# vtuber-plan/vcvits

Measured on AMD Instinct MI355X. Metric: training utterances/sec (gen+disc step) at base.json segment_size, higher is better.
Workload: dtype f32; 1 GPU; configs/base.json widths, HiFi-GAN generator + MPD(8 periods+S) + MSD + STFT/mel-L1, G step + D step + AdamW (learning rate 0: weights held at their seeded initial values); per_gpu_batch=16, global_batch=16, segment_size=16384, parallelism=dp1, process_group_ranks=1, graph_recording_steps_before_warmup=3

## Files before the change

include/vcvits_hip.h:

```cpp
#ifndef VCVITS_HIP_H
#define VCVITS_HIP_H

#include <stdint.h>

#ifdef __cplusplus
extern "C" {
#endif

#define VCV_OK 0
#define VCV_EINVAL (-1)
#define VCV_EHIP (-2)
#define VCV_ELDS (-3)

#define VCV_ACT_NONE 0
#define VCV_ACT_LEAKY 1
#define VCV_ACT_RELU 2
#define VCV_ACT_TANH 3
#define VCV_ACT_LOGCLAMP 4

#define VCV_TF_NONE 0
#define VCV_TF_LEAKY 1
#define VCV_TF_DLEAKY 2
#define VCV_TF_DRELU 3
#define VCV_TF_DTANH 4
// ... 71 lines not shown

typedef struct VcvWgradArgs {
  const float* a;
  const float* b;
  const float* aaux;
  const float* baux;
  float* dw;
  int32_t B, G, Cg, Mg;
  int32_t Ta, Tb, P;
  int32_t K;
  int32_t s, dj, off;
  int32_t a_tf, b_tf;
  int32_t transpose_out;
  float alpha, slope;
  float* dbias;
  float* slab;
  int64_t slab_floats;
  int32_t split_terms;
} VcvWgradArgs;

int vcv_conv_wgrad(const VcvWgradArgs* args, void* stream);
int vcv_conv_wgrad_takes_dma(const VcvWgradArgs* args);
int vcv_conv_wgrad_split_terms(const VcvWgradArgs* args);

int64_t vcv_wgrad_bf16_scratch(const VcvWgradArgs* args);
int vcv_wgrad_bf16(const VcvWgradArgs* args, float* scratch, int64_t scratch_floats, void* stream);
int64_t vcv_wgrad_x3_scratch(const VcvWgradArgs* args);
int vcv_wgrad_x3(const VcvWgradArgs* args, float* scratch, int64_t scratch_floats, void* stream);
int vcv_wgrad_bf16_set_force(int cand, int z);

int vcv_conv_m1_fwd(const float* x, const float* w, const float* bias, float* y, int B, int C, int Tin,
                    int Tout, int P, int K, int stride, int dil, int pad, int in_leaky, int out_act,
                    float slope, void* stream);
int vcv_conv_c1_fwd(const float* x, const float* w, const float* bias, float* y, int B, int M, int Tin, int Tout,
                    int P, int K, int stride, int dil, int pad, int out_act, float slope, void* stream);
int vcv_conv_c1_fwd_masked(const float* x, const float* w, const float* bias, float* y, const float* oaux, int B, int M,
                           int Tin, int Tout, int P, int K, int stride, int dil, int pad, int out_act, float slope,
                           void* stream);
int vcv_conv_c1_fwd_flip(const float* x, const float* w, const float* bias, float* y, const float* oaux, int B, int M, int Tin,
                         int Tout, int P, int K, int stride, int dil, int pad, int out_act, float slope, int flip_taps,
                         void* stream);
int vcv_conv_c1_dgrad(const float* dy, const float* w, float* dx, int B, int M, int Tin, int Tout, int P, int K,
                      int stride, int dil, int pad, void* stream);
int vcv_linear_t1_fwd(const float* x, const float* w, const float* bias, float* y, int B, int C, int M, void* stream);
int vcv_linear_t1_dgrad(const float* dy, const float* w, float* dx, int B, int C, int M, void* stream);
int vcv_linear_t1_wgrad(const float* dy, const float* x, float* dw, int B, int C, int M, void* stream);
// ... 235 lines not shown
```

vcvits_amd/_lib.py:

```python
import ctypes
import os

import torch

_HERE = os.path.dirname(os.path.abspath(__file__))
from . import tuning

LIB_PATH = tuning.text("VCVITS_HIP_LIB", "", "path of another build of libvcvits_hip.so (A/B builds)") or \
    os.path.join(_HERE, "csrc", "libvcvits_hip.so")

VCV_OK = 0
ACT_NONE, ACT_LEAKY, ACT_RELU, ACT_TANH, ACT_LOGCLAMP = 0, 1, 2, 3, 4
TF_NONE, TF_LEAKY, TF_DLEAKY, TF_DRELU, TF_DTANH, TF_DLOGCLAMP = 0, 1, 2, 3, 4, 5

_f32p = ctypes.c_void_p
_i32 = ctypes.c_int32


class VcvConvArgs(ctypes.Structure):
    _fields_ = [
        ("x", _f32p), ("w", _f32p), ("bias", _f32p), ("res", _f32p), ("mask", _f32p),
        ("xaux", _f32p), ("oaux", _f32p), ("y", _f32p),
        ("B", _i32), ("G", _i32), ("Cg", _i32), ("Mg", _i32),
        ("Tin", _i32), ("Tout", _i32), ("P", _i32),
# ... 40 lines not shown


def lib():
    global _lib
    if _lib is None:
        if not os.path.exists(LIB_PATH):
            raise RuntimeError(
                "libvcvits_hip.so not found at %s -- run `python -m vcvits_amd.build_ext` "
                "(there is no CPU fallback for the vcvits hot path)" % LIB_PATH)
        L = ctypes.CDLL(LIB_PATH)
        L.vcv_version.restype = ctypes.c_char_p
        for name in EXPORTS:
            fn = getattr(L, name)
            if name != "vcv_version":
                fn.restype = (ctypes.c_int64 if name in ("vcv_conv_dma_workspace", "vcv_wgrad_bf16_scratch", "vcv_wgrad_x3_scratch", "vcv_layernorm_c_bwd_scratch", "vcv_resblock_pair_supported",
                                                                "vcv_rel_attn_stream_bwd_workspace")
                              else ctypes.c_void_p if name == "vcv_get_seed_offset_ptr" else ctypes.c_int)
                fn.argtypes = _ARGTYPES[name]
        _lib = L
    return _lib


EXPORTS = [
    "vcv_version", "vcv_conv_gemm", "vcv_conv_wgrad", "vcv_conv_wgrad_takes_dma", "vcv_conv_wgrad_split_terms", "vcv_bias_grad",
    "vcv_weight_norm_fwd", "vcv_weight_norm_bwd", "vcv_spectral_norm_fwd", "vcv_spectral_norm_bwd", "vcv_avg3", "vcv_scale", "vcv_mask_mul",
    "vcv_reflect_pad_fwd", "vcv_reflect_pad_bwd", "vcv_avgpool4_fwd", "vcv_avgpool4_bwd",
    "vcv_loss_sum", "vcv_loss_grad", "vcv_adamw", "vcv_stft_mag_fwd", "vcv_stft_mag_bwd",
    "vcv_wn_gate_fwd", "vcv_wn_gate_bwd", "vcv_row_sum", "vcv_wn_res_skip_fwd", "vcv_wn_res_skip_bwd",
    "vcv_split_sample_fwd", "vcv_split_sample_bwd", "vcv_coupling", "vcv_layernorm_c_fwd",
    "vcv_layernorm_c_bwd", "vcv_rel_softmax_fwd", "vcv_rel_value_fwd", "vcv_rel_softmax_bwd",
    "vcv_kl_fwd", "vcv_kl_bwd", "vcv_nearest_fwd", "vcv_nearest_bwd", "vcv_nearest_raw_fwd", "vcv_nearest_raw_bwd", "vcv_slice_fwd", "vcv_slice_bwd",
    "vcv_dropout", "vcv_prof_begin", "vcv_prof_end", "vcv_prof_dump", "vcv_conv_m1_fwd", "vcv_conv_c1_fwd", "vcv_conv_c1_fwd_masked", "vcv_conv_c1_fwd_flip", "vcv_conv_c1_dgrad", "vcv_linear_t1_fwd", "vcv_linear_t1_dgrad", "vcv_linear_t1_wgrad", "vcv_thin_wgrad", "vcv_weight_flip_transpose",
    "vcv_act_grad", "vcv_act_grad_add", "vcv_weight_norm_many_fwd", "vcv_weight_norm_many_bwd", "vcv_loss_many_sum", "vcv_loss_many_grad", "vcv_conv_dma_workspace", "vcv_conv_dma", "vcv_conv_dma_plan", "vcv_conv_dma_run", "vcv_stft_complex_fwd", "vcv_istft", "vcv_grouped41_fwd", "vcv_grouped41_fwd_bf16", "vcv_grouped41_dgrad", "vcv_grouped41_dgrad_bf16", "vcv_grouped41_wgrad", "vcv_grouped41_wgrad_bf16",
    "vcv_prior_sample", "vcv_prof_bytes", "vcv_conv_bf16_plan", "vcv_conv_bf16_run", "vcv_wgrad_bf16_scratch", "vcv_wgrad_bf16", "vcv_act_grad_bias", "vcv_conv_pk_plan", "vcv_conv_pk_run",
    "vcv_conv_x3_plan", "vcv_conv_x3_run", "vcv_conv_x3_set_terms", "vcv_conv_x3_get_terms", "vcv_conv_x3_set_all", "vcv_wgrad_x3_scratch", "vcv_wgrad_x3", "vcv_rel_attn_supported", "vcv_rel_attn_fwd", "vcv_rel_attn_bwd", "vcv_rel_attn_bwd2", "vcv_set_deterministic", "vcv_get_deterministic", "vcv_prof_roof", "vcv_prof_pause", "vcv_conv_x3_pack_job", "vcv_conv_pk_pack_job", "vcv_conv_bf16_pack_job", "vcv_pack_many", "vcv_upload_table",
    "vcv_conv_bf16io_plan", "vcv_conv_bf16io_run", "vcv_cast_f32_x16", "vcv_cast_x16_f32", "vcv_conv_m1_x16_fwd",
    "vcv_prof_active", "vcv_set_seed_offset_ptr", "vcv_get_seed_offset_ptr", "vcv_pack_many_prepared", "vcv_adamw_dev", "vcv_set_words", "vcv_tuning_set", "vcv_tuning_get", "vcv_embedding_t_fwd", "vcv_embedding_t_fwd_checked", "vcv_embedding_t_bwd", "vcv_conv_x3_set_variant", "vcv_conv_plan_describe", "vcv_wgrad_bf16_set_force", "vcv_layernorm_c_bwd_scratch", "vcv_layernorm_c_bwd_ws", "vcv_resblock_pair_supported", "vcv_resblock_pair_pack", "vcv_resblock_pair_x16",
    "vcv_pyin_yin", "vcv_pyin_obs", "vcv_pyin_viterbi",
    "vcv_resample_table", "vcv_resample_apply", "vcv_phase_vocoder", "vcv_istft_ordered",
    "vcv_hubert_bias_gelu", "vcv_hubert_groupnorm_gelu", "vcv_hubert_layernorm_c_gelu", "vcv_hubert_attn_supported", "vcv_hubert_attn_fwd",
    "vcv_hubert_groupnorm_gelu_len", "vcv_hubert_mask_frames", "vcv_hubert_attn_fwd_len",
    "vcv_rel_attn_stream_supported", "vcv_rel_attn_stream_fwd",
    "vcv_rel_attn_stream_train_fwd", "vcv_rel_attn_stream_bwd_workspace", "vcv_rel_attn_stream_bwd",
    "vcv_rel_attn_stream_fwd_bf16", "vcv_hubert_attn_fwd_bf16", "vcv_hubert_attn_fwd_len_bf16",
]


_P, _I, _L, _F, _D = ctypes.c_void_p, ctypes.c_int, ctypes.c_int64, ctypes.c_float, ctypes.c_double
_ARGTYPES = {
    "vcv_conv_gemm": [ctypes.POINTER(VcvConvArgs), _P],
    "vcv_conv_wgrad": [ctypes.POINTER(VcvWgradArgs), _P],
    "vcv_conv_wgrad_takes_dma": [ctypes.POINTER(VcvWgradArgs)],
    "vcv_conv_wgrad_split_terms": [ctypes.POINTER(VcvWgradArgs)],
    "vcv_bias_grad": [_P, _P, _P, _I, _I, _I, _I, _F, _I, _P],
    "vcv_weight_norm_fwd": [_P, _P, _P, _P, _I, _I, _P],
    "vcv_weight_norm_bwd": [_P, _P, _P, _P, _P, _P, _I, _I, _P],
    "vcv_spectral_norm_fwd": [_P, _P, _P, _P, _P, _P, _I, _I, _I, _F, _P],
    "vcv_spectral_norm_bwd": [_P, _P, _P, _P, _P, _P, _P, _I, _I, _P],
    "vcv_avg3": [_P, _P, _P, _P, _L, _P],
    "vcv_scale": [_P, _P, _F, _L, _P],
    "vcv_mask_mul": [_P, _P, _P, _I, _I, _I, _P],
    "vcv_reflect_pad_fwd": [_P, _P, _I, _I, _I, _P],
    "vcv_reflect_pad_bwd": [_P, _P, _I, _I, _I, _P],
    "vcv_avgpool4_fwd": [_P, _P, _I, _I, _P],
    "vcv_avgpool4_bwd": [_P, _P, _I, _I, _P],
    "vcv_loss_sum": [_P, _P, _F, _I, _F, _P, _L, _P],
    "vcv_loss_grad": [_P, _P, _F, _I, _F, _P, _P, _I, _L, _P],
    "vcv_adamw": [_P, _P, _P, _P, _L, _F, _F, _F, _F, _F, _I, _P],
    "vcv_stft_mag_fwd": [_P, _P, _P, _P, _I, _I, _I, _I, _I, _I, _F, _P],
    "vcv_stft_mag_bwd": [_P, _P, _P, _P, _P, _I, _I, _I, _I, _I, _I, _F, _P],
    "vcv_wn_gate_fwd": [_P, _P, _I, _I, _P, _I, _I, _I, _P],
    "vcv_wn_gate_bwd": [_P, _P, _I, _I, _P, _P, _I, _I, _I, _P],
    "vcv_row_sum": [_P, _P, _I, _I, _I, _I, _I, _P],
    "vcv_wn_res_skip_fwd": [_P, _P, _P, _P, _P, _P, _I, _I, _I, _I, _P],
    "vcv_wn_res_skip_bwd": [_P, _P, _P, _P, _P, _I, _I, _I, _P],
    "vcv_split_sample_fwd": [_P, _P, _P, _P, _P, _P, _I, _I, _I, _P],
# ... 250 lines not shown
```

vcvits_amd/csrc/tuning.h:

```cpp
#pragma once

struct VcvTuning {
  int xcd_remap = 1;
  int pk_ws = 1;
  int pk_ws_bf16 = 0;
  int pk_x4 = 1;
  int pk_vec = 1;
  int x3_variant = -1;
  int x3_v6 = 1;
  int x3_js2 = 1;
  int x3_merge_phases = 1;
  int x3_old_ks = 0;
  int x3_all = 0;
  int x3_terms = 6;
  int wgrad_dma = 1;
  int wgrad_tile = -1;
  int wgrad_verbose = 0;
  int wgrad_dma_split = 1;
  int wgrad_bf16_ws = 1;
  int wgrad_finish_vec = 1;
  int bias_rows = 1;
  int c1_chunk = 0;
  int m1_lds = 1;
  int c1_wgrad_pairs = 1;
  int thin_wgrad_wgs = 2048;
  int act_grad_vec = 1;
  int ln_regs = 1;
  int stft_wave = 1;
  int attn_rows = 1;
  int zero_memset = 0;
  int pack_tile = 1;
  int pack_tile_bf16 = 1;
  int pair_dbg = 0;
  int pair_grid = 0;
  int pair_stream = 1;
  int deterministic = 0;
};

VcvTuning& vcv_tuning();
extern "C" int vcv_tuning_set(const char* key, int value);
extern "C" int vcv_tuning_get(const char* key, int* value);
// ... 1 lines not shown
```

vcvits_amd/csrc/version.hip:

```cpp
#include "common.h"
#include <cstring>
extern "C" const char* vcv_version(void) {
  return "vcvits_hip gfx950 fp32-mfma(32x32x2) conv family; built " __DATE__ " " __TIME__;
}

extern "C" int vcv_set_deterministic(int on) {
  vcv_tuning().deterministic = on ? 1 : 0;
  return VCV_OK;
}
extern "C" int vcv_get_deterministic(void) { return vcv_tuning().deterministic; }

namespace {
struct TuningKey { const char* name; int VcvTuning::*field; };
#define TK(f) {#f, &VcvTuning::f}
const TuningKey kTuningKeys[] = {
    TK(xcd_remap), TK(pk_ws), TK(pk_ws_bf16), TK(pk_x4), TK(pk_vec), TK(x3_variant), TK(x3_v6), TK(x3_js2), TK(x3_merge_phases), TK(x3_old_ks), TK(x3_all),
    TK(x3_terms), TK(wgrad_dma), TK(wgrad_tile), TK(wgrad_verbose), TK(wgrad_dma_split), TK(wgrad_bf16_ws), TK(wgrad_finish_vec), TK(bias_rows),
    TK(c1_chunk), TK(m1_lds), TK(c1_wgrad_pairs), TK(thin_wgrad_wgs), TK(act_grad_vec), TK(ln_regs), TK(stft_wave), TK(attn_rows),
    TK(zero_memset), TK(pack_tile), TK(pack_tile_bf16), TK(pair_dbg), TK(pair_grid), TK(pair_stream), TK(deterministic)};
#undef TK
int VcvTuning::*find_key(const char* key, size_t len) {
  for (const TuningKey& k : kTuningKeys)
    if (strlen(k.name) == len && strncmp(k.name, key, len) == 0) return k.field;
  return nullptr;
}
VcvTuning make_tuning() {
  VcvTuning t;
  const char* det = getenv("VCVITS_DETERMINISTIC");
  if (det && det[0] == '1') t.deterministic = 1;
  const char* e = getenv("VCVITS_TUNING");
  while (e && *e) {
    const char* end = strchr(e, ',');
    const size_t n = end ? (size_t)(end - e) : strlen(e);
    const char* eq = (const char*)memchr(e, '=', n);
    if (eq) {
      int VcvTuning::*f = find_key(e, (size_t)(eq - e));
      if (f) t.*f = atoi(eq + 1);
      else fprintf(stderr, "vcvits_hip: VCVITS_TUNING: unknown key '%.*s'\n", (int)(eq - e), e);
    } else if (n) {
      fprintf(stderr, "vcvits_hip: VCVITS_TUNING: '%.*s' is not key=value\n", (int)n, e);
// ... 31 lines not shown
```

vcvits_amd/csrc/wgrad_dma.hip:

```cpp
#include "common.h"
#include "prof.h"
#include "split_terms.h"
#include <cstring>
#include <unordered_map>

namespace {

constexpr int BU = 64, AP = BU + 4, MAXX = 12, TABN = BU + 32;

struct WgGeom {
  int NCH, CP, emin, G4, nmt, nnt, Z, nchunk_u, buf_floats, a_floats, tab_floats;
  float invG4, invP;
};

template <int OFF>
__device__ __forceinline__ f32x4 lds_rd128(unsigned addr) {
  f32x4 v;
  asm volatile("ds_read_b128 %0, %1 offset:%2" : "=v"(v) : "v"(addr), "n"(OFF) : "memory");
  return v;
}
__device__ __forceinline__ float lds_rd32(unsigned addr) {
  float v;
  asm volatile("ds_read_b32 %0, %1" : "=v"(v) : "v"(addr) : "memory");
  return v;
}
__device__ __forceinline__ void lds_wait() { asm volatile("s_waitcnt lgkmcnt(0)" ::: "memory"); }
__device__ __forceinline__ void pin(f32x4& f) { asm volatile("" : "+v"(f)); }
__device__ __forceinline__ void pin(float& f) { asm volatile("" : "+v"(f)); }
__device__ __forceinline__ void pin(bf16x8& f) { asm volatile("" : "+v"(f)); }
template <typename T, int N>
__device__ __forceinline__ void pin(T (&f)[N]) {
#pragma unroll
  for (int i = 0; i < N; ++i) pin(f[i]);
}
__device__ __forceinline__ void divmod(int n, int d, float inv, int& q, int& r) {
  q = (int)((float)n * inv);
  r = n - q * d;
  if (r < 0) r += d, --q;
  if (r >= d) r -= d, ++q;
}
__device__ __forceinline__ f32x4 ld128(__amdgpu_buffer_rsrc_t r, unsigned voff) {
  return __builtin_bit_cast(f32x4, __builtin_amdgcn_raw_buffer_load_b128(r, voff, 0, 0));
}

__device__ __forceinline__ void split_frag(const float (&f)[8], bf16x8 (&t)[3]) {
#pragma unroll
  for (int e = 0; e < 8; ++e) {
    __bf16 t0, t1, t2;
    split3(f[e], t0, t1, t2);
    t[0][e] = t0, t[1][e] = t1, t[2][e] = t2;
  }
}

template <int TM, int TN, int WM, int WN, bool LA, bool LB, bool BIAS, bool STR, int ST>
__global__ void __launch_bounds__(64 * (WM * WN + (WM * WN >= 8 ? 4 : 2)))
wgrad_dma_kernel(const VcvWgradArgs p, const WgGeom tg) {
  constexpr int BM = 32 * TM * WM, BN = 32 * TN * WN, NW = WM * WN, NP = NW >= 8 ? 4 : 2;
  constexpr int MAXA = BM / (4 * NP);
  extern __shared__ float smem[];
  const int tid = threadIdx.x, lane = tid & 63;
  const int wave = __builtin_amdgcn_readfirstlane(tid >> 6);
  const int l31 = lane & 31, h = lane >> 5;

  const int nt = blockIdx.x, mt = blockIdx.y, z = blockIdx.z;
  const int K = p.K, Cg = p.Cg, Mg = p.Mg, P = p.P;
  const int N = Cg * K;
  const int n0 = nt * BN, m0 = mt * BM;
  const int cfirst = n0 / K;
  const int CP = tg.CP, NCH = tg.NCH;
  const unsigned lds0 = (unsigned)(size_t)(__attribute__((address_space(3))) float*)smem;
  const int U = p.Ta * P, TbP = p.Tb * P;
  const int total = p.B * tg.nchunk_u;
  if (z >= total) return;
  auto xspan0 = [&](int uc0) __attribute__((always_inline)) {
    return STR ? ((uc0 / P) * p.s + tg.emin) * P : uc0 + tg.emin * P;
  };

  if (wave >= NW) {
    const int pw = wave - NW;
    __builtin_amdgcn_s_setprio(3);
    f32x4 ra[MAXA], rx[MAXX];
    const int ngx = NCH * tg.G4;
    int xld[MAXX], xi4[MAXX];
    unsigned xst[MAXX];
#pragma unroll
    for (int t = 0; t < MAXX; ++t) {
      const int idx = (t * NP + pw) * 64 + lane;
      int cl, i4;
      divmod(idx, tg.G4, tg.invG4, cl, i4);
      xi4[t] = 4 * i4;
      xld[t] = idx < ngx ? cl * TbP + 4 * i4 : 0x20000000;
      xst[t] = (unsigned)(idx < ngx ? tg.a_floats + cl * CP + 4 * i4 : tg.a_floats + tg.tab_floats + NCH * CP) * 4u;
    }
    if (STR && pw == 1 && lane < TABN - BU) {
      asm volatile("ds_write_b32 %0, %1" ::"v"(lds0 + (unsigned)(tg.a_floats + NCH * CP + BU + lane) * 4u), "v"(0) : "memory");
      asm volatile("ds_write_b32 %0, %1" ::"v"(lds0 + (unsigned)(tg.buf_floats + tg.a_floats + NCH * CP + BU + lane) * 4u), "v"(0)
                   : "memory");
    }
    auto store = [&](int ch, int buf) __attribute__((always_inline)) {
      const int b = ch / tg.nchunk_u;
      const int uc0 = (ch - b * tg.nchunk_u) * BU;
      const unsigned base = lds0 + (unsigned)(buf * tg.buf_floats) * 4u;
      const bool tail = uc0 + BU > U;
#pragma unroll
      for (int t = 0; t < MAXA; ++t) {
        const int row = (t * NP + pw) * 4 + (lane >> 4), c4 = lane & 15;
        f32x4 v = ra[t];
        if (tail) {
          const int nv = U - uc0 - 4 * c4;
#pragma unroll
          for (int e = 0; e < 4; ++e) v[e] = e < nv ? v[e] : 0.f;
        }
        asm volatile("ds_write_b128 %0, %1" ::"v"(base + (unsigned)(row * AP + 4 * c4) * 4u), "v"(v) : "memory");
      }
      const int f0 = xspan0(uc0), f0a = f0 & ~3;
      if (STR && pw == 0) {
        int q, pc;
        divmod(uc0 + lane, P, tg.invP, q, pc);
        const int off = ((q - uc0 / P) * p.s * P + pc + (f0 - f0a)) * 4;
        asm volatile("ds_write_b32 %0, %1" ::"v"(base + (unsigned)(tg.a_floats + NCH * CP + lane) * 4u), "v"(uc0 + lane < U ? off : 0)
                     : "memory");
      }
      const bool edge = f0a < 0 || f0a + 4 * tg.G4 > TbP;
#pragma unroll
      for (int t = 0; t < MAXX; ++t) {
        if ((t * NP + pw) * 64 < ngx) {
          f32x4 v = rx[t];
          if (edge) {
            const int f = f0a + xi4[t];
#pragma unroll
            for (int e = 0; e < 4; ++e) v[e] = (unsigned)(f + e) < (unsigned)TbP ? v[e] : 0.f;
          }
          asm volatile("ds_write_b128 %0, %1" ::"v"(base + xst[t]), "v"(v) : "memory");
        }
      }
    };
// ... 11 lines not shown
      __amdgpu_buffer_rsrc_t rX = __builtin_amdgcn_make_buffer_rsrc((void*)(p.b + ((size_t)b * Cg + cfirst) * (size_t)TbP), 0,
                                                                    (int)((size_t)(Cg - cfirst) * TbP * 4), 0x00020000);
#pragma unroll
      for (int t = 0; t < MAXX; ++t)
        if ((t * NP + pw) * 64 < ngx) {
          unsigned voff = (unsigned)(xld[t] + f0a) * 4u;
          asm volatile("" : "+v"(voff));
          rx[t] = ld128(rX, voff);
        }
    };
    load(z);
    store(z, 0);
    if (z + tg.Z < total) load(z + tg.Z);
    int bufi = 0;
    for (int ch = z; ch < total; ch += tg.Z) {
      lds_wait();
      __syncthreads();
      if (ch + tg.Z < total) {
        store(ch + tg.Z, bufi ^ 1);
        if (ch + 2 * tg.Z < total) load(ch + 2 * tg.Z);
      }
      bufi ^= 1;
    }
    return;
  }

  const int wm = wave / WN, wn = wave % WN;
  unsigned aofs[TM], nofs[TN];
#pragma unroll
  for (int tm = 0; tm < TM; ++tm) aofs[tm] = (unsigned)(((wm * TM + tm) * 32 + l31) * AP + 4 * h) * 4u;
#pragma unroll
  for (int tn = 0; tn < TN; ++tn) {
    int n = n0 + (wn * TN + tn) * 32 + l31;
    if (n > N - 1) n = N - 1;
    const int c = n / K, kw = n - c * K;
    const int e = kw * p.dj + p.off - tg.emin;
    nofs[tn] = (unsigned)(tg.a_floats + (c - cfirst) * CP + e * P + (STR ? 0 : ((tg.emin * P) & 3) + 4 * h)) * 4u;
  }
  const unsigned tabofs = (unsigned)(tg.a_floats + NCH * CP + 4 * h) * 4u;

  f32x16 acc[TM][TN];
#pragma unroll
  for (int tm = 0; tm < TM; ++tm)
#pragma unroll
    for (int tn = 0; tn < TN; ++tn)
#pragma unroll
      for (int e = 0; e < 16; ++e) acc[tm][tn][e] = 0.f;
  const bool do_bias = BIAS && nt == 0 && wn == 0;
  float bsum[TM];
#pragma unroll
  for (int tm = 0; tm < TM; ++tm) bsum[tm] = 0.f;

  int bufi = 0;
  for (int ch = z; ch < total; ch += tg.Z) {
    __syncthreads();
    const unsigned base = lds0 + (unsigned)(bufi * tg.buf_floats) * 4u;
    const int uc0 = (ch % tg.nchunk_u) * BU;
    const int rem = U - uc0;
    const int npair = rem >= BU ? BU / 16 : (rem + 15) >> 4;
    unsigned aad[TM], bad[TN], tad = base + tabofs;
#pragma unroll
    for (int tm = 0; tm < TM; ++tm) aad[tm] = base + aofs[tm];
#pragma unroll
    for (int tn = 0; tn < TN; ++tn) bad[tn] = base + nofs[tn];


    if constexpr (ST == 6) {
      f32x4 a0[TM], a1[TM], b0[TN], b1[TN], t0, t1;
      float b0s[TN][4], b1s[TN][4];
      auto rd_group = [&]() __attribute__((always_inline)) {
        if (STR) t0 = lds_rd128<0>(tad), t1 = lds_rd128<32>(tad);
#pragma unroll
        for (int tm = 0; tm < TM; ++tm) a0[tm] = lds_rd128<0>(aad[tm]), a1[tm] = lds_rd128<32>(aad[tm]);
        if (STR) {
          asm volatile("s_waitcnt lgkmcnt(%0)" ::"n"(2 * TM) : "memory");
          pin(t0), pin(t1);
        }
#pragma unroll
        for (int tn = 0; tn < TN; ++tn) {
          if (!STR) {
            b0[tn] = lds_rd128<0>(bad[tn]), b1[tn] = lds_rd128<32>(bad[tn]);
          } else {
#pragma unroll
            for (int e = 0; e < 4; ++e) b0s[tn][e] = lds_rd32(bad[tn] + __float_as_uint(t0[e]));
#pragma unroll
            for (int e = 0; e < 4; ++e) b1s[tn][e] = lds_rd32(bad[tn] + __float_as_uint(t1[e]));
          }
        }
      };
      auto settle = [&]() __attribute__((always_inline)) {
        lds_wait();
        pin(a0), pin(a1);
        if (STR) {
#pragma unroll
          for (int tn = 0; tn < TN; ++tn)
#pragma unroll
            for (int e = 0; e < 4; ++e) pin(b0s[tn][e]), pin(b1s[tn][e]);
        } else {
          pin(b0), pin(b1);
        }
      };
      rd_group();
      settle();
      for (int pr = 0; pr < npair; ++pr) {
        bf16x8 ap[TM][3], bp[TN][3];
#pragma unroll
        for (int tm = 0; tm < TM; ++tm) {
          float f[8];
#pragma unroll
          for (int e = 0; e < 4; ++e) f[e] = a0[tm][e], f[4 + e] = a1[tm][e];
          if (LA) {
#pragma unroll
            for (int e = 0; e < 8; ++e) f[e] = fmaxf(f[e], f[e] * p.slope);
          }
          if (BIAS && do_bias) bsum[tm] += ((f[0] + f[1]) + (f[2] + f[3])) + ((f[4] + f[5]) + (f[6] + f[7]));
          split_frag(f, ap[tm]);
        }
#pragma unroll
        for (int tn = 0; tn < TN; ++tn) {
          float f[8];
#pragma unroll
          for (int e = 0; e < 4; ++e) f[e] = STR ? b0s[tn][e] : b0[tn][e], f[4 + e] = STR ? b1s[tn][e] : b1[tn][e];
          if (LB) {
#pragma unroll
            for (int e = 0; e < 8; ++e) f[e] = fmaxf(f[e], f[e] * p.slope);
          }
          split_frag(f, bp[tn]);
        }
#pragma unroll
        for (int pl = 0; pl < 3; ++pl) {
#pragma unroll
          for (int tm = 0; tm < TM; ++tm) pin(ap[tm][pl]);
#pragma unroll
          for (int tn = 0; tn < TN; ++tn) pin(bp[tn][pl]);
        }
#pragma unroll
        for (int tm = 0; tm < TM; ++tm) aad[tm] += 64;
        if (!STR) {
#pragma unroll
          for (int tn = 0; tn < TN; ++tn) bad[tn] += 64;
        }
        tad += 64;
        if (pr + 1 < npair) rd_group();
        mma_product<6>(acc, ap, bp);
        settle();
      }
      bufi ^= 1;
      continue;
    }
    f32x4 a0[TM], a1[TM], b0[TN], b1[TN], t0, t1;
    float b0s[TN][4], b1s[TN][4];
#define WG_LOAD(A, Bf, T, OFF)                                                                  \
  {                                                                                             \
    _Pragma("unroll") for (int tm = 0; tm < TM; ++tm) A[tm] = lds_rd128<OFF>(aad[tm]);          \
    if (!STR) {                                                                                 \
      _Pragma("unroll") for (int tn = 0; tn < TN; ++tn) Bf[tn] = lds_rd128<OFF>(bad[tn]);       \
    } else {                                                                                    \
      _Pragma("unroll") for (int tn = 0; tn < TN; ++tn) _Pragma("unroll") for (int e = 0; e < 4; ++e)  \
          Bf##s[tn][e] = lds_rd32(bad[tn] + __float_as_uint(T[e]));                             \
    }                                                                                           \
// ... 77 lines not shown
        else unsafeAtomicAdd(p.dw + (size_t)ml * N + n, p.alpha * acc[tm][tn][e]);
      }
    }
  }
}

__global__ void __launch_bounds__(256) wgrad_slab_finish_kernel(const float* __restrict__ slab, float* __restrict__ dw,
                                                                size_t n, int Z, float alpha) {
  const size_t i = (size_t)blockIdx.x * 256 + threadIdx.x;
  if (i >= n) return;
  float s = slab[i];
  for (int z = 1; z < Z; ++z) s += slab[(size_t)z * n + i];
  dw[i] += alpha * s;
}

template <int TM, int TN, int WM, int WN, bool STR, int ST>
void (*pick_kernel_st(const VcvWgradArgs& a))(const VcvWgradArgs, const WgGeom) {
  const bool la = a.a_tf == VCV_TF_LEAKY, lb = a.b_tf == VCV_TF_LEAKY;
  return la ? (lb ? wgrad_dma_kernel<TM, TN, WM, WN, true, true, false, STR, ST> : wgrad_dma_kernel<TM, TN, WM, WN, true, false, false, STR, ST>)
            : (a.dbias ? (lb ? wgrad_dma_kernel<TM, TN, WM, WN, false, true, true, STR, ST> : wgrad_dma_kernel<TM, TN, WM, WN, false, false, true, STR, ST>)
                       : (lb ? wgrad_dma_kernel<TM, TN, WM, WN, false, true, false, STR, ST> : wgrad_dma_kernel<TM, TN, WM, WN, false, false, false, STR, ST>));
}
template <int TM, int TN, int WM, int WN, bool STR>
void (*pick_kernel(const VcvWgradArgs& a, bool split))(const VcvWgradArgs, const WgGeom) {
  return split ? pick_kernel_st<TM, TN, WM, WN, STR, 6>(a) : pick_kernel_st<TM, TN, WM, WN, STR, 0>(a);
}

constexpr double SPLIT_SHAPE[7] = {1.0, 0.83, 0.65, 0.73, 0.67, 0.57, 0.57};
constexpr double SPLIT_BASE = 0.85;

bool wanted_split(const VcvWgradArgs& a) { return (long long)a.B * a.Ta * a.P >= 1024; }

bool takes_split(const VcvWgradArgs& a) {
  const VcvTuning& t = vcv_tuning();
  return a.split_terms == 6 && t.wgrad_dma_split != 0 && t.x3_terms == 6 && (t.x3_all != 0 || wanted_split(a));
}

struct WgPlan {
  WgGeom g;
  size_t lds;
  double cost;
};

template <int TM, int TN, int WM, int WN, bool STR>
WgPlan plan(const VcvWgradArgs& a, bool split) {
  constexpr int BM = 32 * TM * WM, BN = 32 * TN * WN, NP = WM * WN >= 8 ? 4 : 2, NT = 64 * (WM * WN + NP);
  WgPlan pl;
  pl.cost = -1.0;
  WgGeom& g = pl.g;
  const int N = a.Cg * a.K;
  g.nnt = vcv_cdiv(N, BN);
  g.nmt = vcv_cdiv(a.Mg, BM);
  g.NCH = (BN - 1) / a.K + 2;
  if (g.NCH > a.Cg + 1) g.NCH = a.Cg + 1;
  const int jspan = (a.K - 1) * a.dj;
  g.emin = a.off + (jspan < 0 ? jspan : 0);
  const int emax = jspan < 0 ? -jspan : jspan;
  const int nq = STR ? (a.P - 1 + BU - 1) / a.P + 1 : 0;
  const int span = STR ? ((nq - 1) * a.s + emax + 1) * a.P : BU + emax * a.P;
  g.G4 = (span + 3 + 3) / 4;
  g.invG4 = 1.0f / (float)g.G4, g.invP = 1.0f / (float)a.P;
  if ((long long)g.NCH * g.G4 > (long long)MAXX * NP * 64) return pl;
  g.a_floats = BM * AP;
  g.tab_floats = TABN;
  int want = (a.K * (emax / (a.K > 1 ? a.K - 1 : 1)) * a.P + 3) / 4 * 4 % 64;
  if (want < 8) want = 8;
  g.CP = 4 * g.G4;
  while (g.CP % 64 != want % 64) g.CP += 4;
  if (g.CP - 4 * g.G4 > 32) g.CP = 4 * g.G4 + 4;
  for (int attempt = 0; attempt < 2; ++attempt) {
    g.buf_floats = g.a_floats + g.NCH * g.CP + g.tab_floats + 16;
    pl.lds = 2ull * g.buf_floats * 4;
    if (pl.lds <= VCV_LDS_LIMIT) break;
    g.CP = 4 * g.G4 + ((4 * g.G4) % 32 == 0 ? 4 : 0);
  }
  if (pl.lds > VCV_LDS_LIMIT) return pl;
  const long long U = (long long)a.Ta * a.P;
  g.nchunk_u = (int)((U + BU - 1) / BU);
  const long long total = (long long)a.B * g.nchunk_u;
  void (*kern)(const VcvWgradArgs, const WgGeom) = pick_kernel<TM, TN, WM, WN, STR>(a, split);
  static int occ_cache[2][2][2][2] = {};
  int& oc = occ_cache[split][a.a_tf == VCV_TF_LEAKY][a.b_tf == VCV_TF_LEAKY][a.dbias != nullptr];
  if (oc == 0) {
    (void)hipFuncSetAttribute((const void*)kern, hipFuncAttributeMaxDynamicSharedMemorySize, VCV_LDS_LIMIT);
    int nb = 0;
    if (hipOccupancyMaxActiveBlocksPerMultiprocessor(&nb, (const void*)kern, NT, 0) != hipSuccess || nb < 1) nb = 1;
    oc = nb;
  }
  long long occ = (long long)(VCV_LDS_LIMIT / pl.lds);
  if (occ > oc) occ = oc;
  if (occ < 1) occ = 1;
  const double shape = BM == 128 ? (BN == 256 ? 1.0 : BN == 128 ? 0.93 : 0.77)
                     : BM == 64  ? (BN == 256 ? 0.905 : BN == 128 ? 0.76 : 0.58)
                                 : 0.62;
  const double shape6 = BM == 128 ? (BN == 256 ? SPLIT_SHAPE[0] : BN == 128 ? SPLIT_SHAPE[1] : SPLIT_SHAPE[2])
                      : BM == 64  ? (BN == 256 ? SPLIT_SHAPE[3] : BN == 128 ? SPLIT_SHAPE[4] : SPLIT_SHAPE[5])
                                  : SPLIT_SHAPE[6];
  const double rate = (split ? SPLIT_BASE * shape6 : 0.70 * shape) * (STR ? 0.93 : 1.0) * 157.3e12 / 256.0;
  const double t_stage = 2.0 * BM * BN * BU / rate * 1e6, t_fix = 4.0;
  const long long tiles = (long long)g.nnt * g.nmt;
  const long long slots = 256 * occ;
  const size_t nw = (size_t)a.Mg * N;
  const long long zcap = a.slab ? (long long)(a.slab_floats / (int64_t)nw) : 1024;
  if (a.slab && zcap < 1) return pl;
  long long Z = 1;
  double best = 1e30;
  for (long long z = 1; z <= total && z <= 1024 && z <= zcap; ++z) {
    const double rounds = (double)((tiles * z + slots - 1) / slots);
    const double r = tiles * z < slots ? (double)(tiles * z) / 256.0 : (double)occ;
    const double share = r <= 1.0 ? (0.3 + 0.7 / (double)occ) * (double)occ : (0.3 + 0.7 * r / (double)occ) * (double)occ;
    const double epi = a.slab ? (double)z * nw * 4.0 * (1.0 / 4e12 + 1.0 / 4e12) * 1e6 + 3.0 : (double)z * nw * 4.0 / 1.3e12 * 1e6;
    const double cost = rounds * ((double)((total + z - 1) / z) * t_stage * share + t_fix) + epi;
    if (cost < best - 1e-9) best = cost, Z = z;
  }
  g.Z = (int)Z;
  pl.cost = best;
  const bool verbose = vcv_tuning().wgrad_verbose != 0;
  if (verbose)
    fprintf(stderr, "wgrad plan M%d C%d K%d U%lld s%d tile %dx%d: occ %lld tiles %lld total %lld Z %lld cost %.1f us lds %zu%s\n", a.Mg, a.Cg, a.K,
            U, a.s, BM, BN, occ, tiles, total, Z, best, pl.lds, split ? " terms 6" : "");
  return pl;
}

template <int TM, int TN, int WM, int WN, bool STR>
int run(const VcvWgradArgs& a, const WgPlan& pl, bool split, hipStream_t st) {
  constexpr int BM = 32 * TM * WM, BN = 32 * TN * WN, NP = WM * WN >= 8 ? 4 : 2, NT = 64 * (WM * WN + NP);
  const WgGeom& g = pl.g;
  void (*kern)(const VcvWgradArgs, const WgGeom) = pick_kernel<TM, TN, WM, WN, STR>(a, split);
  if (pl.lds > 64 * 1024 && hipFuncSetAttribute((const void*)kern, hipFuncAttributeMaxDynamicSharedMemorySize, (int)pl.lds) != hipSuccess)
    return VCV_EHIP;
  const int N = a.Cg * a.K;
  const size_t nw = (size_t)a.Mg * N;
  dim3 grid(g.nnt, g.nmt, g.Z), block(NT);
  const double flops = 2.0 * a.B * a.Mg * a.Cg * a.K * a.P * (double)a.Ta;
  const int tag[12] = {a.B, split ? 4 : 1, a.Cg, a.Mg, a.K, a.Ta, a.P, a.s, g.Z, 2, BM * 1000 + BN, g.G4};
  hipEvent_t ev0, ev1;
  const double abytes = 4.0 * ((double)a.B * a.Mg * a.Ta * a.P + (double)a.B * a.Cg * a.Tb * a.P + (double)a.Mg * a.Cg * a.K);
  if (split) vcv_prof_events(VCV_PROF_WGRAD_DMA, flops, tag, 12, &ev0, &ev1, abytes, 6 * flops / VCV_PEAK_BF16_MFMA);
  else vcv_prof_events(VCV_PROF_WGRAD_DMA, flops, tag, 12, &ev0, &ev1, abytes);
  VCV_LAUNCH_EV(kern, grid, block, (unsigned)pl.lds, st, ev0, ev1, a, g);
  if (a.slab)
    hipLaunchKernelGGL(wgrad_slab_finish_kernel, dim3((unsigned)((nw + 255) / 256)), dim3(256), 0, st, (const float*)a.slab, a.dw,
                       nw, g.Z, a.alpha);
  return vcv_check_launch();
}

#define WG_TILES(X) X(0, 2, 2, 2, 4) X(1, 2, 1, 2, 4) X(2, 1, 1, 4, 2) X(3, 1, 2, 2, 4) X(4, 1, 2, 2, 2) X(5, 1, 1, 2, 2) X(6, 1, 2, 1, 2)

struct PlanKey {
  int v[16];
  int64_t slab;
  bool operator==(const PlanKey& o) const { return memcmp(v, o.v, sizeof(v)) == 0 && slab == o.slab; }
};
struct PlanKeyHash {
  size_t operator()(const PlanKey& k) const {
    uint64_t h = 1469598103934665603ull ^ (uint64_t)k.slab;
    for (int i = 0; i < 16; ++i) h = (h ^ (uint64_t)(uint32_t)k.v[i]) * 1099511628211ull;
    return (size_t)h;
  }
};
struct PlanEntry { WgPlan pl; int which; };

template <bool STR>
int launch(const VcvWgradArgs& a, hipStream_t st) {
  const int only = vcv_tuning().wgrad_tile;
  const bool split = takes_split(a);
  static thread_local std::unordered_map<PlanKey, PlanEntry, PlanKeyHash> cache;
  const PlanKey key = {{a.B, a.Cg, a.Mg, a.Ta, a.Tb, a.P, a.K, a.s, a.dj, a.off, a.a_tf, a.b_tf, a.dbias != nullptr, a.slab != nullptr,
                        split, only},
                       a.slab ? a.slab_floats : 0};
  auto hit = cache.find(key);
  WgPlan best;
  best.cost = -1.0;
  int which = -1;
  if (hit != cache.end()) best = hit->second.pl, which = hit->second.which;
  else {
#define WG_PLAN(I, TM, TN, WM, WN)                                                        \
  if ((only < 0 || only == I) && a.Mg >= 32 * TM * WM / 2 + 1 || (I == 6 && which < 0)) { \
    const WgPlan pl = plan<TM, TN, WM, WN, STR>(a, split);                                \
    if (pl.cost >= 0.0 && (which < 0 || pl.cost < best.cost)) best = pl, which = I;       \
  }
  WG_TILES(WG_PLAN)
#undef WG_PLAN
    if (cache.size() > 4096) cache.clear();
    cache[key] = PlanEntry{best, which};
  }
  if (which < 0) return -100;
#define WG_RUN(I, TM, TN, WM, WN) \
  if (which == I) return run<TM, TN, WM, WN, STR>(a, best, split, st);
  WG_TILES(WG_RUN)
#undef WG_RUN
  return -100;
}

}

static bool wgrad_dma_eligible(const VcvWgradArgs& a) {
  const bool tf_ok = (a.a_tf == VCV_TF_NONE || a.a_tf == VCV_TF_LEAKY) && (a.b_tf == VCV_TF_NONE || a.b_tf == VCV_TF_LEAKY) &&
                     a.slope >= 0.f && a.slope < 1.f;
  const int N = a.Cg * a.K;
  const long long U = (long long)a.Ta * a.P;
  if (a.G != 1 || !tf_ok || a.transpose_out || a.Mg < 32 || N < 96 || U < 64 || a.s < 1 || a.s > 8) return false;
  if ((long long)a.Mg * U * 4 >= (1ll << 31) || (long long)a.Cg * a.Tb * a.P * 4 >= (1ll << 31)) return false;
  return true;
}

int vcv_wgrad_dma_try(const VcvWgradArgs& a, hipStream_t st) {
  if (!wgrad_dma_eligible(a)) return -100;
  return a.s == 1 ? launch<false>(a, st) : launch<true>(a, st);
}

extern "C" int vcv_conv_wgrad_takes_dma(const VcvWgradArgs* a) {
  return a && vcv_tuning().wgrad_dma != 0 && wgrad_dma_eligible(*a) ? 1 : 0;
}

extern "C" int vcv_conv_wgrad_split_terms(const VcvWgradArgs* a) {
  return vcv_conv_wgrad_takes_dma(a) && takes_split(*a) ? 6 : 0;
}
```

vcvits_amd/tuning.py:

```python
import os

REGISTRY = {}


def _declare(name, kind, default, doc, value):
    REGISTRY[name] = (kind, default, doc, value)
    return value


def flag(name, default, doc):
    raw = os.environ.get(name)
    return _declare(name, "flag", default, doc, default if raw is None else raw == "1")


def integer(name, default, doc):
    raw = os.environ.get(name)
    return _declare(name, "int", default, doc, default if raw is None else int(raw))


def number(name, default, doc):
    raw = os.environ.get(name)
    return _declare(name, "float", default, doc, default if raw is None else float(raw))


def text(name, default, doc):
    return _declare(name, "text", default, doc, os.environ.get(name, default))


def live_flag(name):
    kind, default, doc, _ = REGISTRY[name]
    raw = os.environ.get(name)
    return default if raw is None else (raw == "1" if kind == "flag" else int(raw))


KERNEL_KEYS = ("xcd_remap", "pk_ws", "pk_ws_bf16", "pk_x4", "pk_vec", "x3_variant", "x3_v6", "x3_js2", "x3_merge_phases", "x3_old_ks", "x3_all", "x3_terms",
               "wgrad_dma", "wgrad_tile", "wgrad_verbose", "wgrad_dma_split", "wgrad_bf16_ws", "wgrad_finish_vec", "bias_rows", "c1_chunk", "m1_lds",
               "c1_wgrad_pairs", "thin_wgrad_wgs", "act_grad_vec", "ln_regs", "stft_wave", "attn_rows", "zero_memset", "pack_tile",
               "pack_tile_bf16", "pair_dbg", "pair_grid", "pair_stream", "deterministic")


def kernel_get(key):
    import ctypes
    from ._lib import check, lib
    v = ctypes.c_int(0)
    check(lib().vcv_tuning_get(key.encode(), ctypes.byref(v)), "vcv_tuning_get(%s)" % key)
    return v.value


def kernel_set(key, value):
    from ._lib import check, lib
    check(lib().vcv_tuning_set(key.encode(), int(value)), "vcv_tuning_set(%s)" % key)


def table():
    import importlib
    for mod in ("vcvits_amd._lib", "vcvits_amd.ops", "vcvits_amd.mel_processing", "vcvits_amd.model.flow", "vcvits_amd.model.modules",
                "vcvits_amd.model.discriminators._pair", "vcvits_amd.light.optim", "vcvits_amd.light.graphed"):
        importlib.import_module(mod)
    out = ["environment variables of the host side (name, default, meaning):"]
# ... 17 lines not shown
```

Measured before the change: 251.8 utterances/s.

## Pre-split A operand into bf16x3 planes in wgrad DMA producer waves

Adds a new kernel form (ST=7) for the DMA weight-gradient kernel, used for small tiles. The producer waves apply leaky activation, split each A element into three bf16 terms and write them to LDS as separate planes, so the MFMA waves read ready-made bf16 fragments instead of converting fp32 on every use. The bias gradient moves into the producer waves, computed with DPP row sums and atomics. The planner takes this form only when it does not lower occupancy versus the existing split form, at the cost of larger LDS for A and extra atomics.

```diff
diff --git a/include/vcvits_hip.h b/include/vcvits_hip.h
--- a/include/vcvits_hip.h
+++ b/include/vcvits_hip.h
@@ -117,6 +117,7 @@
 int vcv_conv_wgrad(const VcvWgradArgs* args, void* stream);
 int vcv_conv_wgrad_takes_dma(const VcvWgradArgs* args);
 int vcv_conv_wgrad_split_terms(const VcvWgradArgs* args);
+int vcv_conv_wgrad_presplit(const VcvWgradArgs* args);
 
 int64_t vcv_wgrad_bf16_scratch(const VcvWgradArgs* args);
 int vcv_wgrad_bf16(const VcvWgradArgs* args, float* scratch, int64_t scratch_floats, void* stream);
diff --git a/vcvits_amd/_lib.py b/vcvits_amd/_lib.py
--- a/vcvits_amd/_lib.py
+++ b/vcvits_amd/_lib.py
@@ -86,7 +86,7 @@
 
 
 EXPORTS = [
-    "vcv_version", "vcv_conv_gemm", "vcv_conv_wgrad", "vcv_conv_wgrad_takes_dma", "vcv_conv_wgrad_split_terms", "vcv_bias_grad",
+    "vcv_version", "vcv_conv_gemm", "vcv_conv_wgrad", "vcv_conv_wgrad_takes_dma", "vcv_conv_wgrad_split_terms", "vcv_conv_wgrad_presplit", "vcv_bias_grad",
     "vcv_weight_norm_fwd", "vcv_weight_norm_bwd", "vcv_spectral_norm_fwd", "vcv_spectral_norm_bwd", "vcv_avg3", "vcv_scale", "vcv_mask_mul",
     "vcv_reflect_pad_fwd", "vcv_reflect_pad_bwd", "vcv_avgpool4_fwd", "vcv_avgpool4_bwd",
     "vcv_loss_sum", "vcv_loss_grad", "vcv_adamw", "vcv_stft_mag_fwd", "vcv_stft_mag_bwd",
@@ -116,6 +116,7 @@
     "vcv_conv_wgrad": [ctypes.POINTER(VcvWgradArgs), _P],
     "vcv_conv_wgrad_takes_dma": [ctypes.POINTER(VcvWgradArgs)],
     "vcv_conv_wgrad_split_terms": [ctypes.POINTER(VcvWgradArgs)],
+    "vcv_conv_wgrad_presplit": [ctypes.POINTER(VcvWgradArgs)],
     "vcv_bias_grad": [_P, _P, _P, _I, _I, _I, _I, _F, _I, _P],
     "vcv_weight_norm_fwd": [_P, _P, _P, _P, _I, _I, _P],
     "vcv_weight_norm_bwd": [_P, _P, _P, _P, _P, _P, _I, _I, _P],
diff --git a/vcvits_amd/csrc/tuning.h b/vcvits_amd/csrc/tuning.h
--- a/vcvits_amd/csrc/tuning.h
+++ b/vcvits_amd/csrc/tuning.h
@@ -17,6 +17,7 @@
   int wgrad_tile = -1;
   int wgrad_verbose = 0;
   int wgrad_dma_split = 1;
+  int wgrad_dma_presplit = 1;
   int wgrad_bf16_ws = 1;
   int wgrad_finish_vec = 1;
   int bias_rows = 1;
diff --git a/vcvits_amd/csrc/version.hip b/vcvits_amd/csrc/version.hip
--- a/vcvits_amd/csrc/version.hip
+++ b/vcvits_amd/csrc/version.hip
@@ -15,7 +15,7 @@
 #define TK(f) {#f, &VcvTuning::f}
 const TuningKey kTuningKeys[] = {
     TK(xcd_remap), TK(pk_ws), TK(pk_ws_bf16), TK(pk_x4), TK(pk_vec), TK(x3_variant), TK(x3_v6), TK(x3_js2), TK(x3_merge_phases), TK(x3_old_ks), TK(x3_all),
-    TK(x3_terms), TK(wgrad_dma), TK(wgrad_tile), TK(wgrad_verbose), TK(wgrad_dma_split), TK(wgrad_bf16_ws), TK(wgrad_finish_vec), TK(bias_rows),
+    TK(x3_terms), TK(wgrad_dma), TK(wgrad_tile), TK(wgrad_verbose), TK(wgrad_dma_split), TK(wgrad_dma_presplit), TK(wgrad_bf16_ws), TK(wgrad_finish_vec), TK(bias_rows),
     TK(c1_chunk), TK(m1_lds), TK(c1_wgrad_pairs), TK(thin_wgrad_wgs), TK(act_grad_vec), TK(ln_regs), TK(stft_wave), TK(attn_rows),
     TK(zero_memset), TK(pack_tile), TK(pack_tile_bf16), TK(pair_dbg), TK(pair_grid), TK(pair_stream), TK(deterministic)};
 #undef TK
diff --git a/vcvits_amd/csrc/wgrad_dma.hip b/vcvits_amd/csrc/wgrad_dma.hip
--- a/vcvits_amd/csrc/wgrad_dma.hip
+++ b/vcvits_amd/csrc/wgrad_dma.hip
@@ -7,6 +7,9 @@
 namespace {
 
 constexpr int BU = 64, AP = BU + 4, MAXX = 12, TABN = BU + 32;
+constexpr int APB = 2 * BU + 16;
+typedef __bf16 bf16x4 __attribute__((ext_vector_type(4)));
+typedef unsigned u32x2 __attribute__((ext_vector_type(2)));
 
 struct WgGeom {
   int NCH, CP, emin, G4, nmt, nnt, Z, nchunk_u, buf_floats, a_floats, tab_floats;
@@ -33,6 +36,11 @@
 #pragma unroll
   for (int i = 0; i < N; ++i) pin(f[i]);
 }
+template <typename T, int N, int M>
+__device__ __forceinline__ void pin(T (&f)[N][M]) {
+#pragma unroll
+  for (int i = 0; i < N; ++i) pin(f[i]);
+}
 __device__ __forceinline__ void divmod(int n, int d, float inv, int& q, int& r) {
   q = (int)((float)n * inv);
   r = n - q * d;
@@ -43,6 +51,17 @@
   return __builtin_bit_cast(f32x4, __builtin_amdgcn_raw_buffer_load_b128(r, voff, 0, 0));
 }
 
+template <int CTRL>
+__device__ __forceinline__ float dpp_add(float s) {
+  return s + __builtin_bit_cast(float, __builtin_amdgcn_update_dpp(0, __builtin_bit_cast(int, s), CTRL, 0xf, 0xf, true));
+}
+__device__ __forceinline__ float row_sum16(float s) {
+  s = dpp_add<0xB1>(s);
+  s = dpp_add<0x4E>(s);
+  s = dpp_add<0x141>(s);
+  return dpp_add<0x140>(s);
+}
+
 __device__ __forceinline__ void split_frag(const float (&f)[8], bf16x8 (&t)[3]) {
 #pragma unroll
   for (int e = 0; e < 8; ++e) {
@@ -57,6 +76,8 @@
 wgrad_dma_kernel(const VcvWgradArgs p, const WgGeom tg) {
   constexpr int BM = 32 * TM * WM, BN = 32 * TN * WN, NW = WM * WN, NP = NW >= 8 ? 4 : 2;
   constexpr int MAXA = BM / (4 * NP);
+  constexpr bool PS = ST == 7;
+  constexpr int PLANE = BM * APB;
   extern __shared__ float smem[];
   const int tid = threadIdx.x, lane = tid & 63;
   const int wave = __builtin_amdgcn_readfirstlane(tid >> 6);
@@ -80,6 +101,8 @@
     const int pw = wave - NW;
     __builtin_amdgcn_s_setprio(3);
     f32x4 ra[MAXA], rx[MAXX];
+    static_assert(MAXA <= 16, "one bias accumulator per lane");
+    float pbs = 0.f;
     const int ngx = NCH * tg.G4;
     int xld[MAXX], xi4[MAXX];
     unsigned xst[MAXX];
@@ -111,7 +134,30 @@
 #pragma unroll
           for (int e = 0; e < 4; ++e) v[e] = e < nv ? v[e] : 0.f;
         }
-        asm volatile("ds_write_b128 %0, %1" ::"v"(base + (unsigned)(row * AP + 4 * c4) * 4u), "v"(v) : "memory");
+        if constexpr (PS) {
+          if (LA) {
+#pragma unroll
+            for (int e = 0; e < 4; ++e) v[e] = fmaxf(v[e], v[e] * p.slope);
+          }
+          if (BIAS && nt == 0) {
+            float rs = row_sum16((v[0] + v[1]) + (v[2] + v[3]));
+            asm volatile("" : "+v"(rs));
+            pbs += c4 == t ? rs : 0.f;
+          }
+          bf16x4 pl[3];
+#pragma unroll
+          for (int e = 0; e < 4; ++e) {
+            __bf16 t0, t1, t2;
+            split3(v[e], t0, t1, t2);
+            pl[0][e] = t0, pl[1][e] = t1, pl[2][e] = t2;
+          }
+          const unsigned ad = base + (unsigned)(row * APB + (c4 >> 2) * 32 + (((c4 & 1) << 1) | ((c4 >> 1) & 1)) * 8);
+          asm volatile("ds_write_b64 %0, %1" ::"v"(ad), "v"(__builtin_bit_cast(u32x2, pl[0])) : "memory");
+          asm volatile("ds_write_b64 %0, %1" ::"v"(ad + (unsigned)PLANE), "v"(__builtin_bit_cast(u32x2, pl[1])) : "memory");
+          asm volatile("ds_write_b64 %0, %1" ::"v"(ad + 2u * (unsigned)PLANE), "v"(__builtin_bit_cast(u32x2, pl[2])) : "memory");
+        } else {
+          asm volatile("ds_write_b128 %0, %1" ::"v"(base + (unsigned)(row * AP + 4 * c4) * 4u), "v"(v) : "memory");
+        }
       }
       const int f0 = xspan0(uc0), f0a = f0 & ~3;
       if (STR && pw == 0) {
@@ -169,13 +215,20 @@
       }
       bufi ^= 1;
     }
+    if constexpr (PS && BIAS) {
+      if (nt == 0) {
+        const int ml = m0 + ((lane & 15) * NP + pw) * 4 + (lane >> 4);
+        if ((lane & 15) < MAXA && ml < Mg) unsafeAtomicAdd(p.dbias + ml, pbs);
+      }
+    }
     return;
   }
 
   const int wm = wave / WN, wn = wave % WN;
   unsigned aofs[TM], nofs[TN];
 #pragma unroll
-  for (int tm = 0; tm < TM; ++tm) aofs[tm] = (unsigned)(((wm * TM + tm) * 32 + l31) * AP + 4 * h) * 4u;
+  for (int tm = 0; tm < TM; ++tm)
+    aofs[tm] = PS ? (unsigned)(((wm * TM + tm) * 32 + l31) * APB + 16 * h) : (unsigned)(((wm * TM + tm) * 32 + l31) * AP + 4 * h) * 4u;
 #pragma unroll
   for (int tn = 0; tn < TN; ++tn) {
     int n = n0 + (wn * TN + tn) * 32 + l31;
@@ -193,7 +246,7 @@
     for (int tn = 0; tn < TN; ++tn)
 #pragma unroll
       for (int e = 0; e < 16; ++e) acc[tm][tn][e] = 0.f;
-  const bool do_bias = BIAS && nt == 0 && wn == 0;
+  const bool do_bias = BIAS && !PS && nt == 0 && wn == 0;
   float bsum[TM];
 #pragma unroll
   for (int tm = 0; tm < TM; ++tm) bsum[tm] = 0.f;
@@ -212,15 +265,19 @@
     for (int tn = 0; tn < TN; ++tn) bad[tn] = base + nofs[tn];
 
 
-    if constexpr (ST == 6) {
+    if constexpr (ST >= 6) {
       f32x4 a0[TM], a1[TM], b0[TN], b1[TN], t0, t1;
+      f32x4 an[TM][3];
       float b0s[TN][4], b1s[TN][4];
       auto rd_group = [&]() __attribute__((always_inline)) {
         if (STR) t0 = lds_rd128<0>(tad), t1 = lds_rd128<32>(tad);
 #pragma unroll
-        for (int tm = 0; tm < TM; ++tm) a0[tm] = lds_rd128<0>(aad[tm]), a1[tm] = lds_rd128<32>(aad[tm]);
+        for (int tm = 0; tm < TM; ++tm) {
+          if constexpr (PS) an[tm][0] = lds_rd128<0>(aad[tm]), an[tm][1] = lds_rd128<PLANE>(aad[tm]), an[tm][2] = lds_rd128<2 * PLANE>(aad[tm]);
+          else a0[tm] = lds_rd128<0>(aad[tm]), a1[tm] = lds_rd128<32>(aad[tm]);
+        }
         if (STR) {
-          asm volatile("s_waitcnt lgkmcnt(%0)" ::"n"(2 * TM) : "memory");
+          asm volatile("s_waitcnt lgkmcnt(%0)" ::"n"((PS ? 3 : 2) * TM) : "memory");
           pin(t0), pin(t1);
         }
 #pragma unroll
@@ -237,7 +294,8 @@
       };
       auto settle = [&]() __attribute__((always_inline)) {
         lds_wait();
-        pin(a0), pin(a1);
+        if constexpr (PS) pin(an);
+        else pin(a0), pin(a1);
         if (STR) {
 #pragma unroll
           for (int tn = 0; tn < TN; ++tn)
@@ -253,6 +311,11 @@
         bf16x8 ap[TM][3], bp[TN][3];
 #pragma unroll
         for (int tm = 0; tm < TM; ++tm) {
+          if constexpr (PS) {
+#pragma unroll
+            for (int pl = 0; pl < 3; ++pl) ap[tm][pl] = __builtin_bit_cast(bf16x8, an[tm][pl]);
+            continue;
+          }
           float f[8];
 #pragma unroll
           for (int e = 0; e < 4; ++e) f[e] = a0[tm][e], f[4 + e] = a1[tm][e];
@@ -282,7 +345,7 @@
           for (int tn = 0; tn < TN; ++tn) pin(bp[tn][pl]);
         }
 #pragma unroll
-        for (int tm = 0; tm < TM; ++tm) aad[tm] += 64;
+        for (int tm = 0; tm < TM; ++tm) aad[tm] += PS ? 32 : 64;
         if (!STR) {
 #pragma unroll
           for (int tn = 0; tn < TN; ++tn) bad[tn] += 64;
@@ -406,8 +469,10 @@
                        : (lb ? wgrad_dma_kernel<TM, TN, WM, WN, false, true, false, STR, ST> : wgrad_dma_kernel<TM, TN, WM, WN, false, false, false, STR, ST>));
 }
 template <int TM, int TN, int WM, int WN, bool STR>
-void (*pick_kernel(const VcvWgradArgs& a, bool split))(const VcvWgradArgs, const WgGeom) {
-  return split ? pick_kernel_st<TM, TN, WM, WN, STR, 6>(a) : pick_kernel_st<TM, TN, WM, WN, STR, 0>(a);
+void (*pick_kernel(const VcvWgradArgs& a, int form))(const VcvWgradArgs, const WgGeom) {
+  if constexpr (TM * TN <= 2 && !STR)
+    if (form == 2) return pick_kernel_st<TM, TN, WM, WN, STR, 7>(a);
+  return form ? pick_kernel_st<TM, TN, WM, WN, STR, 6>(a) : pick_kernel_st<TM, TN, WM, WN, STR, 0>(a);
 }
 
 constexpr double SPLIT_SHAPE[7] = {1.0, 0.83, 0.65, 0.73, 0.67, 0.57, 0.57};
@@ -419,6 +484,8 @@
   const VcvTuning& t = vcv_tuning();
   return a.split_terms == 6 && t.wgrad_dma_split != 0 && t.x3_terms == 6 && (t.x3_all != 0 || wanted_split(a));
 }
+
+bool offers_presplit() { return vcv_tuning().wgrad_dma_presplit != 0; }
 
 struct WgPlan {
   WgGeom g;
@@ -427,7 +494,8 @@
 };
 
 template <int TM, int TN, int WM, int WN, bool STR>
-WgPlan plan(const VcvWgradArgs& a, bool split) {
+WgPlan plan(const VcvWgradArgs& a, int form) {
+  const bool split = form != 0;
   constexpr int BM = 32 * TM * WM, BN = 32 * TN * WN, NP = WM * WN >= 8 ? 4 : 2, NT = 64 * (WM * WN + NP);
   WgPlan pl;
   pl.cost = -1.0;
@@ -445,7 +513,7 @@
   g.G4 = (span + 3 + 3) / 4;
   g.invG4 = 1.0f / (float)g.G4, g.invP = 1.0f / (float)a.P;
   if ((long long)g.NCH * g.G4 > (long long)MAXX * NP * 64) return pl;
-  g.a_floats = BM * AP;
+  g.a_floats = form == 2 ? 3 * BM * APB / 4 : BM * AP;
   g.tab_floats = TABN;
   int want = (a.K * (emax / (a.K > 1 ? a.K - 1 : 1)) * a.P + 3) / 4 * 4 % 64;
   if (want < 8) want = 8;
@@ -462,18 +530,28 @@
   const long long U = (long long)a.Ta * a.P;
   g.nchunk_u = (int)((U + BU - 1) / BU);
   const long long total = (long long)a.B * g.nchunk_u;
-  void (*kern)(const VcvWgradArgs, const WgGeom) = pick_kernel<TM, TN, WM, WN, STR>(a, split);
-  static int occ_cache[2][2][2][2] = {};
-  int& oc = occ_cache[split][a.a_tf == VCV_TF_LEAKY][a.b_tf == VCV_TF_LEAKY][a.dbias != nullptr];
-  if (oc == 0) {
-    (void)hipFuncSetAttribute((const void*)kern, hipFuncAttributeMaxDynamicSharedMemorySize, VCV_LDS_LIMIT);
-    int nb = 0;
-    if (hipOccupancyMaxActiveBlocksPerMultiprocessor(&nb, (const void*)kern, NT, 0) != hipSuccess || nb < 1) nb = 1;
-    oc = nb;
-  }
-  long long occ = (long long)(VCV_LDS_LIMIT / pl.lds);
-  if (occ > oc) occ = oc;
-  if (occ < 1) occ = 1;
+  static int occ_cache[3][2][2][2] = {};
+  auto by_registers = [&](int f) {
+    int& oc = occ_cache[f][a.a_tf == VCV_TF_LEAKY][a.b_tf == VCV_TF_LEAKY][a.dbias != nullptr];
+    if (oc == 0) {
+      void (*kern)(const VcvWgradArgs, const WgGeom) = pick_kernel<TM, TN, WM, WN, STR>(a, f);
+      (void)hipFuncSetAttribute((const void*)kern, hipFuncAttributeMaxDynamicSharedMemorySize, VCV_LDS_LIMIT);
+      int nb = 0;
+      if (hipOccupancyMaxActiveBlocksPerMultiprocessor(&nb, (const void*)kern, NT, 0) != hipSuccess || nb < 1) nb = 1;
+      oc = nb;
+    }
+    return (long long)oc;
+  };
+  auto held = [&](int f, size_t lds) {
+    long long occ = (long long)(VCV_LDS_LIMIT / lds);
+    if (occ > by_registers(f)) occ = by_registers(f);
+    return occ < 1 ? 1 : occ;
+  };
+  const long long occ = held(form, pl.lds);
+  if (form == 2) {
+    const size_t lds1 = pl.lds - 2ull * 4 * (size_t)(g.a_floats - BM * AP);
+    if (TM * TN > 2 || occ < held(1, lds1)) return pl;
+  }
   const double shape = BM == 128 ? (BN == 256 ? 1.0 : BN == 128 ? 0.93 : 0.77)
                      : BM == 64  ? (BN == 256 ? 0.905 : BN == 128 ? 0.76 : 0.58)
                                  : 0.62;
@@ -507,10 +585,11 @@
 }
 
 template <int TM, int TN, int WM, int WN, bool STR>
-int run(const VcvWgradArgs& a, const WgPlan& pl, bool split, hipStream_t st) {
+int run(const VcvWgradArgs& a, const WgPlan& pl, int form, hipStream_t st) {
+  const bool split = form != 0;
   constexpr int BM = 32 * TM * WM, BN = 32 * TN * WN, NP = WM * WN >= 8 ? 4 : 2, NT = 64 * (WM * WN + NP);
   const WgGeom& g = pl.g;
-  void (*kern)(const VcvWgradArgs, const WgGeom) = pick_kernel<TM, TN, WM, WN, STR>(a, split);
+  void (*kern)(const VcvWgradArgs, const WgGeom) = pick_kernel<TM, TN, WM, WN, STR>(a, form);
   if (pl.lds > 64 * 1024 && hipFuncSetAttribute((const void*)kern, hipFuncAttributeMaxDynamicSharedMemorySize, (int)pl.lds) != hipSuccess)
     return VCV_EHIP;
   const int N = a.Cg * a.K;
@@ -543,35 +622,43 @@
     return (size_t)h;
   }
 };
-struct PlanEntry { WgPlan pl; int which; };
+struct PlanEntry { WgPlan pl; int which, form; };
 
 template <bool STR>
-int launch(const VcvWgradArgs& a, hipStream_t st) {
+PlanEntry lookup(const VcvWgradArgs& a) {
   const int only = vcv_tuning().wgrad_tile;
-  const bool split = takes_split(a);
+  const bool split = takes_split(a), presplit = split && offers_presplit();
   static thread_local std::unordered_map<PlanKey, PlanEntry, PlanKeyHash> cache;
   const PlanKey key = {{a.B, a.Cg, a.Mg, a.Ta, a.Tb, a.P, a.K, a.s, a.dj, a.off, a.a_tf, a.b_tf, a.dbias != nullptr, a.slab != nullptr,
-                        split, only},
+                        split + presplit, only},
                        a.slab ? a.slab_floats : 0};
   auto hit = cache.find(key);
   WgPlan best;
   best.cost = -1.0;
-  int which = -1;
-  if (hit != cache.end()) best = hit->second.pl, which = hit->second.which;
-  else {
+  int which = -1, form = 0;
+  if (hit != cache.end()) return hit->second;
+  {
 #define WG_PLAN(I, TM, TN, WM, WN)                                                        \
   if ((only < 0 || only == I) && a.Mg >= 32 * TM * WM / 2 + 1 || (I == 6 && which < 0)) { \
-    const WgPlan pl = plan<TM, TN, WM, WN, STR>(a, split);                                \
-    if (pl.cost >= 0.0 && (which < 0 || pl.cost < best.cost)) best = pl, which = I;       \
+    int f = split ? (presplit && !STR && TM * TN <= 2 ? 2 : 1) : 0;                       \
+    WgPlan pl = plan<TM, TN, WM, WN, STR>(a, f);                                          \
+    if (f == 2 && pl.cost < 0.0) pl = plan<TM, TN, WM, WN, STR>(a, f = 1);                \
+    if (pl.cost >= 0.0 && (which < 0 || pl.cost < best.cost)) best = pl, which = I, form = f; \
   }
   WG_TILES(WG_PLAN)
 #undef WG_PLAN
     if (cache.size() > 4096) cache.clear();
-    cache[key] = PlanEntry{best, which};
-  }
-  if (which < 0) return -100;
+    cache[key] = PlanEntry{best, which, form};
+  }
+  return PlanEntry{best, which, form};
+}
+
+template <bool STR>
+int launch(const VcvWgradArgs& a, hipStream_t st) {
+  const PlanEntry e = lookup<STR>(a);
+  if (e.which < 0) return -100;
 #define WG_RUN(I, TM, TN, WM, WN) \
-  if (which == I) return run<TM, TN, WM, WN, STR>(a, best, split, st);
+  if (e.which == I) return run<TM, TN, WM, WN, STR>(a, e.pl, e.form, st);
   WG_TILES(WG_RUN)
 #undef WG_RUN
   return -100;
@@ -601,3 +688,9 @@
 extern "C" int vcv_conv_wgrad_split_terms(const VcvWgradArgs* a) {
   return vcv_conv_wgrad_takes_dma(a) && takes_split(*a) ? 6 : 0;
 }
+
+extern "C" int vcv_conv_wgrad_presplit(const VcvWgradArgs* a) {
+  if (vcv_conv_wgrad_split_terms(a) != 6) return 0;
+  const PlanEntry e = a->s == 1 ? lookup<false>(*a) : lookup<true>(*a);
+  return e.which >= 0 && e.form == 2 ? 1 : 0;
+}
diff --git a/vcvits_amd/tuning.py b/vcvits_amd/tuning.py
--- a/vcvits_amd/tuning.py
+++ b/vcvits_amd/tuning.py
@@ -34,7 +34,7 @@
 
 
 KERNEL_KEYS = ("xcd_remap", "pk_ws", "pk_ws_bf16", "pk_x4", "pk_vec", "x3_variant", "x3_v6", "x3_js2", "x3_merge_phases", "x3_old_ks", "x3_all", "x3_terms",
-               "wgrad_dma", "wgrad_tile", "wgrad_verbose", "wgrad_dma_split", "wgrad_bf16_ws", "wgrad_finish_vec", "bias_rows", "c1_chunk", "m1_lds",
+               "wgrad_dma", "wgrad_tile", "wgrad_verbose", "wgrad_dma_split", "wgrad_dma_presplit", "wgrad_bf16_ws", "wgrad_finish_vec", "bias_rows", "c1_chunk", "m1_lds",
                "c1_wgrad_pairs", "thin_wgrad_wgs", "act_grad_vec", "ln_regs", "stft_wave", "attn_rows", "zero_memset", "pack_tile",
                "pack_tile_bf16", "pair_dbg", "pair_grid", "pair_stream", "deterministic")
 
```

Result: no change. 252.8 utterances/s (median of 6 runs) (+0.4%).
